# ipastore/glue-factory-colon

Measured on AMD Instinct MI355X. Metric: image-pairs/sec (SuperPoint+LightGlue, 1024 kpts, 640x480), higher is better.
Workload: dtype f32; 1 GPU; SuperPoint-open + LightGlue, 1024 kpts, 640x480 synthetic pairs (BASELINE.json configs[1]); keypoints=1024, parallelism=dp1 (pairs sharded, one final gather), weights=name-seeded seed 0 (no network), pairs_gathered=32, rccl_ranks=1

## Files before the change

### glue-factory-colon_amd/csrc/conv_wino.hip

```cpp
#include "common.h"

#define WT_Y 16
#define WT_X 8
#define WP_R 18
#define WP_C 12
#define WKC 16
#define WPATCH (WP_R * WP_C * WKC)
#define WIM_R 20
#define WIM_C 12
#ifndef WINO_DIAG
#define WINO_DIAG 0
#endif

struct WinoArgs {
  const float* x;
  const float* w;
  const float* bias;
  const float* scale;
  const float* shift;
  float* y;
  int B, H, W, cin, cout, relu;
  int tiles_x, tiles_y;
  const float* w1;
  const float* b1;
  const float* s1;
  const float* t1;
  int xcd_remap;
#if WINO_DIAG & 256
  unsigned long long* diag;
#endif
};
#if WINO_DIAG & 256
static unsigned long long* g_wino_diag = nullptr;
extern "C" void gfc_diag_set_wino_stamps(void* p) { g_wino_diag = (unsigned long long*)p; }
#define WINO_T(v_) const unsigned long long v_ = __builtin_readcyclecounter()
#else
#define WINO_T(v_) do {} while (0)
#endif

__global__ void pack_conv3x3_wino_kernel(const float* __restrict__ w, float* __restrict__ out, int cout, int cin) {
  const int idx = blockIdx.x * blockDim.x + threadIdx.x;
  if (idx >= cout * cin) return;
  const int ci = idx % cin, co = idx / cin;
  double g[3][3];
  for (int r = 0; r < 3; ++r)
    for (int c = 0; c < 3; ++c) g[r][c] = (double)w[((size_t)co * cin + ci) * 9 + r * 3 + c];
  const double G[4][3] = {{1.0, 0.0, 0.0}, {0.5, 0.5, 0.5}, {0.5, -0.5, 0.5}, {0.0, 0.0, 1.0}};
  double t[4][3];
  for (int i = 0; i < 4; ++i)
    for (int c = 0; c < 3; ++c) t[i][c] = G[i][0] * g[0][c] + G[i][1] * g[1][c] + G[i][2] * g[2][c];
  const int nb = co / 64, nt = (co % 64) / 32, l31 = co % 32;
  const int kg = ci / 8, h = (ci % 8) / 4, s = ci % 4;
  const int lane = 32 * h + l31;
  for (int xi = 0; xi < 4; ++xi)
    for (int nu = 0; nu < 4; ++nu) {
      const double u = t[xi][0] * G[nu][0] + t[xi][1] * G[nu][1] + t[xi][2] * G[nu][2];
      const size_t o = ((((((size_t)nb * 4 + xi) * (cin / 8) + kg) * 4 + nu) * 2 + nt) * 64 + lane) * 4 + s;
      out[o] = (float)u;
    }
}

extern "C" int gfc_pack_conv3x3_wino(const float* w_oihw, float* w_packed, int cout, int cin, void* stream) {
  if (!w_oihw || !w_packed || cout <= 0 || cin <= 0 || cout % 64 || cin % WKC) return GFC_ERR_INVALID;
  const int total = cout * cin;
  hipLaunchKernelGGL(pack_conv3x3_wino_kernel, dim3((total + 255) / 256), dim3(256), 0, (hipStream_t)stream, w_oihw,
                     w_packed, cout, cin);
  GFC_LAUNCH_CHECK();
  return GFC_OK;
}

__device__ __forceinline__ float4 f4_axpy(float s, float4 a, float4 b) {
  return make_float4(fmaf(s, a.x, b.x), fmaf(s, a.y, b.y), fmaf(s, a.z, b.z), fmaf(s, a.w, b.w));
}
__device__ __forceinline__ float4 f4_add(float4 a, float4 b) { return make_float4(a.x + b.x, a.y + b.y, a.z + b.z, a.w + b.w); }
__device__ __forceinline__ float4 f4_sub(float4 a, float4 b) { return make_float4(a.x - b.x, a.y - b.y, a.z - b.z, a.w - b.w); }

template <bool POOL, bool STEM>
__global__ __launch_bounds__(256, 2) void conv3x3_wino_kernel(WinoArgs a) {
  extern __shared__ __attribute__((aligned(16))) float smem[];
  float* in_s = smem;
  float* img_s = smem + 16384;
  float* c1_s = img_s + WIM_R * WIM_C;

  const int tid = threadIdx.x, lane = tid & 63;
  const int xi = __builtin_amdgcn_readfirstlane(tid >> 6);
  const int l31 = lane & 31, h = lane >> 5;
  const int cin = a.cin, nchunks = cin / WKC;

  const int ntiles = a.tiles_x * a.tiles_y * a.B;
  const int nitems = ntiles * (a.cout / 64);
  const int nbpair = (a.cout / 64) % 2 == 0 ? 2 : 1;
  int item = blockIdx.x;
  int x0, y0, b, nb;
  const float* xin;
  const float4* wp;
#define WINO_DECODE(w_, x0_, y0_, b_, nb_, xin_, wp_)                                              \
  do {                                                                                             \
    unsigned l_ = a.xcd_remap ? gfc_xcd_chunk((unsigned)(w_), (unsigned)nitems) : (unsigned)(w_);  \
    const int lo_ = (int)(l_ % (unsigned)nbpair);                                                  \
    l_ /= (unsigned)nbpair;                                                                        \
    int t_ = (int)(l_ % (unsigned)ntiles);                                                         \
    nb_ = (int)(l_ / (unsigned)ntiles) * nbpair + lo_;                                             \
    x0_ = (t_ % a.tiles_x) * WT_X;                                                                 \
    t_ /= a.tiles_x;                                                                               \
    y0_ = (t_ % a.tiles_y) * WT_Y;                                                                 \
    b_ = t_ / a.tiles_y;                                                                           \
    xin_ = a.x + (size_t)b_ * a.H * a.W * (STEM ? 1 : cin);                                        \
    wp_ = reinterpret_cast<const float4*>(a.w) + (((size_t)nb_ * 4 + xi) * (cin / 8)) * 512;        \
  } while (0)
  WINO_DECODE(item, x0, y0, b, nb, xin, wp);

  float4 ireg[3];
  int st_off[3];
  int st_gofs[3];
#pragma unroll
  for (int i = 0; i < 3; ++i) {
    const int idx = tid + 256 * i;
    const int pix = idx >> 2, c4 = idx & 3;
    const int py = pix / 10, px = pix - py * 10;
    const int R = (py >> 1) + (py & 1) * 9, C = (px >> 1) + (px & 1) * 5;
    st_off[i] = idx < 720 ? (R * WP_C + C) * WKC + ((c4 ^ (R & 3)) << 2) : -1;
  }
#define WINO_GOFS(y0_, x0_)                                                                        \
  _Pragma("unroll") for (int i_ = 0; i_ < 3; ++i_) {                                               \
    const int py_ = ((tid + 256 * i_) >> 2) / 10, px_ = ((tid + 256 * i_) >> 2) - py_ * 10;        \
    const int gy_ = (y0_) - 1 + py_, gx_ = (x0_) - 1 + px_;                                        \
    const bool in_ = st_off[i_] >= 0 && gy_ >= 0 && gy_ < a.H && gx_ >= 0 && gx_ < a.W;            \
    if constexpr (STEM) st_gofs[i_] = in_ ? (py_ * WIM_C + px_) : -1;  \
    else st_gofs[i_] = in_ ? (int)(((size_t)gy_ * a.W + gx_) * cin + ((tid & 3) << 2)) : -1;       \
  }
#define WINO_LOAD_IN(xin_, chunk_)                                                                \
  _Pragma("unroll") for (int i_ = 0; i_ < 3; ++i_) {                                               \
    float4 v_ = make_float4(0.f, 0.f, 0.f, 0.f);                                                   \
    if (st_gofs[i_] >= 0) v_ = *reinterpret_cast<const float4*>((xin_) + st_gofs[i_] + (chunk_) * WKC); \
    ireg[i_] = v_;                                                                                 \
  }
#define WINO_FILL_IN(chunk_)                                                                      \
  {                                                                                                \
                     \
    const int c0_ = (chunk_) * WKC + ((tid & 3) << 2);                                             \
    float4 wv_[9];                                                                                 \
    _Pragma("unroll") for (int t2_ = 0; t2_ < 9; ++t2_)                                            \
        wv_[t2_] = *reinterpret_cast<const float4*>(c1_s + t2_ * 64 + c0_);                        \
    const float4 b1_ = *reinterpret_cast<const float4*>(c1_s + 576 + c0_);                         \
    const float4 s1_ = *reinterpret_cast<const float4*>(c1_s + 640 + c0_);                         \
    const float4 t1_ = *reinterpret_cast<const float4*>(c1_s + 704 + c0_);                         \
    _Pragma("unroll") for (int i_ = 0; i_ < 3; ++i_) {                                             \
      float4 v_ = make_float4(0.f, 0.f, 0.f, 0.f);   \
      if (st_gofs[i_] >= 0) {                                                                      \
        const float* ip_ = img_s + st_gofs[i_];                                                    \
        _Pragma("unroll") for (int t2_ = 0; t2_ < 9; ++t2_) {                                      \
          const float f_ = ip_[(t2_ / 3) * WIM_C + t2_ % 3];                                       \
          v_.x = fmaf(f_, wv_[t2_].x, v_.x); v_.y = fmaf(f_, wv_[t2_].y, v_.y);                    \
          v_.z = fmaf(f_, wv_[t2_].z, v_.z); v_.w = fmaf(f_, wv_[t2_].w, v_.w);                    \
        }                                                                                          \
        v_.x = fmaxf(v_.x + b1_.x, 0.f) * s1_.x + t1_.x; v_.y = fmaxf(v_.y + b1_.y, 0.f) * s1_.y + t1_.y; \
        v_.z = fmaxf(v_.z + b1_.z, 0.f) * s1_.z + t1_.z; v_.w = fmaxf(v_.w + b1_.w, 0.f) * s1_.w + t1_.w; \
      }                                                                                            \
      ireg[i_] = v_;                                                                               \
    }                                                                                              \
  }
#define WINO_STORE_IN(buf_)                                                                       \
  _Pragma("unroll") for (int i_ = 0; i_ < 3; ++i_)                                                 \
    if (st_off[i_] >= 0) *reinterpret_cast<float4*>(in_s + (buf_) * WPATCH + st_off[i_]) = ireg[i_];
#define WINO_IMG(xin_, y0_, x0_)                                                                   \
  ((tid < WIM_R * WIM_C && (y0_) - 2 + tid / WIM_C >= 0 && (y0_) - 2 + tid / WIM_C < a.H &&        \
    (x0_) - 2 + tid % WIM_C >= 0 && (x0_) - 2 + tid % WIM_C < a.W)                                 \
       ? (xin_)[(size_t)((y0_) - 2 + tid / WIM_C) * a.W + (x0_) - 2 + tid % WIM_C] : 0.f)

  WINO_GOFS(y0, x0);
  if constexpr (STEM) {
    if (tid < WIM_R * WIM_C) img_s[tid] = WINO_IMG(xin, y0, x0);
    for (int i = tid; i < 768; i += 256)
      c1_s[i] = i < 576 ? a.w1[i] : i < 640 ? a.b1[i - 576] : i < 704 ? (a.s1 ? a.s1[i - 640] : 1.f)
                                                                         : (a.t1 ? a.t1[i - 704] : 0.f);
    __syncthreads();
    WINO_FILL_IN(0);
  } else {
    WINO_LOAD_IN(xin, 0);
  }
  float4 bq[4][2];
#pragma unroll
  for (int nu = 0; nu < 4; ++nu)
#pragma unroll
    for (int nt = 0; nt < 2; ++nt) bq[nu][nt] = wp[(nu * 2 + nt) * 64 + lane];

  const int a1 = xi == 0 ? 0 : xi == 2 ? 2 : 1;
  const int a2 = xi == 0 ? 2 : xi == 1 ? 2 : xi == 2 ? 1 : 3;
  const float sg = xi == 1 ? 1.f : -1.f;
  const int ty = l31 >> 2, tx = l31 & 3;
  const int R1 = ty + (a1 >> 1) + (a1 & 1) * 9, R2 = ty + (a2 >> 1) + (a2 & 1) * 9;
  const int o1 = (R1 * WP_C + tx) * WKC + ((h ^ (R1 & 3)) << 2);
  const int o2 = (R2 * WP_C + tx) * WKC + ((h ^ (R2 & 3)) << 2);

#if WINO_DIAG & 256
  unsigned long long d_k = 0, d_x = 0, d_s = 0, d_n = 0, d_epi10 = 0;
  const unsigned long long d_t0 = __builtin_readcyclecounter();
#endif
  while (true) {
  WINO_T(t_a);
  WINO_STORE_IN(0);
  __syncthreads();
  f32x16 acc[4][2];
#pragma unroll
  for (int nu = 0; nu < 4; ++nu)
#pragma unroll
    for (int nt = 0; nt < 2; ++nt)
#pragma unroll
      for (int r = 0; r < 16; ++r) acc[nu][nt][r] = 0.f;
  const int next_item = item + gridDim.x;
  const bool more = !STEM && next_item < nitems;
  int nx0 = 0, ny0 = 0, nbb = 0, nnb = 0;
  const float* nxin = xin;
  const float4* nwp = wp;
  if (more) WINO_DECODE(next_item, nx0, ny0, nbb, nnb, nxin, nwp);

  for (int c = 0; c < nchunks; ++c) {
    const bool has_next = c + 1 < nchunks;
    const float* ps = in_s + (c & 1) * WPATCH;
#pragma unroll
    for (int g = 0; g < 2; ++g) {
      const float* p1 = ps + (g ? (o1 ^ 8) : o1);
      const float* p2 = ps + (g ? (o2 ^ 8) : o2);
      const float4 t0 = f4_axpy(sg, *reinterpret_cast<const float4*>(p2), *reinterpret_cast<const float4*>(p1));
      const float4 t1 = f4_axpy(sg, *reinterpret_cast<const float4*>(p2 + 5 * WKC), *reinterpret_cast<const float4*>(p1 + 5 * WKC));
      const float4 t2 = f4_axpy(sg, *reinterpret_cast<const float4*>(p2 + 1 * WKC), *reinterpret_cast<const float4*>(p1 + 1 * WKC));
      const float4 t3 = f4_axpy(sg, *reinterpret_cast<const float4*>(p2 + 6 * WKC), *reinterpret_cast<const float4*>(p1 + 6 * WKC));
      float4 v[4];
      v[0] = f4_sub(t0, t2);
      v[1] = f4_add(t1, t2);
      v[2] = f4_sub(t2, t1);
      v[3] = f4_sub(t1, t3);
      const int kg_next = 2 * c + g + 1;
      const bool more_b = kg_next < cin / 8 || more;
      const float4* bsrc = kg_next < cin / 8 ? wp + (size_t)kg_next * 512 : nwp;
#pragma unroll
      for (int nu = 0; nu < 4; ++nu) {
        acc[nu][0] = mfma32(v[nu].x, bq[nu][0].x, acc[nu][0]);
        acc[nu][1] = mfma32(v[nu].x, bq[nu][1].x, acc[nu][1]);
        acc[nu][0] = mfma32(v[nu].y, bq[nu][0].y, acc[nu][0]);
        acc[nu][1] = mfma32(v[nu].y, bq[nu][1].y, acc[nu][1]);
        acc[nu][0] = mfma32(v[nu].z, bq[nu][0].z, acc[nu][0]);
        acc[nu][1] = mfma32(v[nu].z, bq[nu][1].z, acc[nu][1]);
        acc[nu][0] = mfma32(v[nu].w, bq[nu][0].w, acc[nu][0]);
        acc[nu][1] = mfma32(v[nu].w, bq[nu][1].w, acc[nu][1]);
        if (more_b) {
          bq[nu][0] = bsrc[(nu * 2 + 0) * 64 + lane];
          bq[nu][1] = bsrc[(nu * 2 + 1) * 64 + lane];
        }
      }
      if (g == 0) {
        if constexpr (STEM) {
          if (has_next) { WINO_FILL_IN(c + 1); }
        } else {
          if (has_next) { WINO_LOAD_IN(xin, c + 1); }
          else if (more) { WINO_GOFS(ny0, nx0); WINO_LOAD_IN(nxin, 0); }
        }
      }
    }
    if (has_next) WINO_STORE_IN((c + 1) & 1);
    __syncthreads();
  }

  WINO_T(t_b);
  float* ex = smem;
#pragma unroll
  for (int nt = 0; nt < 2; ++nt)
#pragma unroll
    for (int r = 0; r < 16; ++r) {
      const float m0 = acc[0][nt][r], m1 = acc[1][nt][r], m2 = acc[2][nt][r], m3 = acc[3][nt][r];
      const int o = acc_row(r, h) * 64 + nt * 32 + l31;
      ex[(xi * 2 + 0) * 2048 + o] = (m0 + m1) + m2;
      ex[(xi * 2 + 1) * 2048 + o] = (m1 - m2) - m3;
    }
  __syncthreads();
  WINO_T(t_c);
  const int q4 = (tid & 15) * 4;
  const int co = nb * 64 + q4;
  const float4 bi = *reinterpret_cast<const float4*>(a.bias + co);
  const float4 sc = a.scale ? *reinterpret_cast<const float4*>(a.scale + co) : make_float4(1.f, 1.f, 1.f, 1.f);
  const float4 sh = a.shift ? *reinterpret_cast<const float4*>(a.shift + co) : make_float4(0.f, 0.f, 0.f, 0.f);
  const bool relu = a.relu != 0;
#pragma unroll
  for (int k = 0; k < 2; ++k) {
    const int tile = (tid >> 4) + 16 * k;
    const float* zp = ex + tile * 64 + q4;
    float4 yv[2][2];
#pragma unroll
    for (int j = 0; j < 2; ++j) {
      const float4 z0 = *reinterpret_cast<const float4*>(zp + (0 * 2 + j) * 2048);
      const float4 z1 = *reinterpret_cast<const float4*>(zp + (1 * 2 + j) * 2048);
      const float4 z2 = *reinterpret_cast<const float4*>(zp + (2 * 2 + j) * 2048);
      const float4 z3 = *reinterpret_cast<const float4*>(zp + (3 * 2 + j) * 2048);
      yv[0][j] = f4_add(f4_add(z0, z1), z2);
      yv[1][j] = f4_sub(f4_sub(z1, z2), z3);
    }
#pragma unroll
    for (int i = 0; i < 2; ++i)
#pragma unroll
      for (int j = 0; j < 2; ++j) {
        float4 t = f4_add(yv[i][j], bi);
        if (relu) t = make_float4(fmaxf(t.x, 0.f), fmaxf(t.y, 0.f), fmaxf(t.z, 0.f), fmaxf(t.w, 0.f));
        yv[i][j] = make_float4(t.x * sc.x + sh.x, t.y * sc.y + sh.y, t.z * sc.z + sh.z, t.w * sc.w + sh.w);
      }
    const int oy = (y0 >> 1) + (tile >> 2), ox = (x0 >> 1) + (tile & 3);
    if constexpr (POOL) {
      const int Ho = a.H >> 1, Wo = a.W >> 1;
      if (oy < Ho && ox < Wo) {
        const float4 u = yv[0][0], v = yv[0][1], w = yv[1][0], z = yv[1][1];
        *reinterpret_cast<float4*>(a.y + (((size_t)b * Ho + oy) * Wo + ox) * a.cout + co) =
            make_float4(fmaxf(fmaxf(u.x, v.x), fmaxf(w.x, z.x)), fmaxf(fmaxf(u.y, v.y), fmaxf(w.y, z.y)),
                        fmaxf(fmaxf(u.z, v.z), fmaxf(w.z, z.z)), fmaxf(fmaxf(u.w, v.w), fmaxf(w.w, z.w)));
      }
    } else {
#pragma unroll
      for (int i = 0; i < 2; ++i)
#pragma unroll
        for (int j = 0; j < 2; ++j) {
          const int gy = 2 * oy + i, gx = 2 * ox + j;
          if (gy < a.H && gx < a.W)
            *reinterpret_cast<float4*>(a.y + (((size_t)b * a.H + gy) * a.W + gx) * a.cout + co) = yv[i][j];
        }
    }
  }
#if WINO_DIAG & 256
  {
    WINO_T(t_d);
    d_k += t_b - t_a; d_x += t_c - t_b; d_s += t_d - t_c; d_n += 1;
    if (d_n == 10) d_epi10 = t_b;
  }
#endif
  if (!more) break;
  item = next_item; x0 = nx0; y0 = ny0; b = nbb; nb = nnb; xin = nxin; wp = nwp;
  __syncthreads();
  }
#if WINO_DIAG & 256
  if (a.diag && lane == 0) {
    unsigned hw, xcc;
    asm volatile("s_getreg_b32 %0, hwreg(HW_REG_HW_ID)" : "=s"(hw));
    asm volatile("s_getreg_b32 %0, hwreg(HW_REG_XCC_ID)" : "=s"(xcc));
    unsigned long long* o = a.diag + ((size_t)blockIdx.x * 4 + xi) * 8;
    o[0] = d_k; o[1] = d_x; o[2] = d_s; o[3] = d_n; o[4] = __builtin_readcyclecounter() - d_t0;
    o[5] = (unsigned long long)hw | ((unsigned long long)(xcc & 0xf) << 32); o[6] = d_t0; o[7] = d_epi10;
  }
#endif
#undef WINO_DECODE
#undef WINO_GOFS
#undef WINO_LOAD_IN
#undef WINO_FILL_IN
#undef WINO_STORE_IN
#undef WINO_IMG
}

template <bool POOL, bool STEM>
static int launch_wino(const WinoArgs& a, hipStream_t st) {
  static_assert(2 * WPATCH <= 16384, "the exchange buffer covers the patch buffers");
  constexpr size_t lds = (size_t)(16384 + (STEM ? WIM_R * WIM_C + 768 : 0)) * sizeof(float);
  static std::atomic<unsigned long long> lds_ok{0};
  if (lds > 64 * 1024) gfc_allow_dynamic_lds((const void*)conv3x3_wino_kernel<POOL, STEM>, lds, lds_ok);
  const long long nitems = (long long)a.tiles_x * a.tiles_y * a.B * (a.cout / 64);
  long long resident = ((long long)gfc_device_cus() * 2) & ~7ll;
  if (resident < 8) resident = 8;
  const long long grid = (STEM || nitems < resident) ? nitems : resident;
  WinoArgs wa = a;
  wa.xcd_remap = nitems >= 16;
#if WINO_DIAG & 256
  wa.diag = g_wino_diag;
#endif
  hipLaunchKernelGGL((conv3x3_wino_kernel<POOL, STEM>), dim3((unsigned)grid), dim3(256), lds, st, wa);
  GFC_LAUNCH_CHECK();
  return GFC_OK;
}

extern "C" int gfc_conv3x3_wino(const float* x, const float* w_wino, const float* bias, const float* scale,
                                const float* shift, float* y, int B, int H, int W, int cin, int cout, int relu, int pool,
                                void* stream) {
  if (!x || !w_wino || !bias || !y || B <= 0 || H <= 0 || W <= 0) return GFC_ERR_INVALID;
  if ((scale == nullptr) != (shift == nullptr)) return GFC_ERR_INVALID;
  if (cin % WKC != 0 || cout % 64 != 0 || cin <= 0 || cout <= 0) return GFC_ERR_UNSUPPORTED;
  if ((long long)H * W * cin >= (1ll << 31)) return GFC_ERR_UNSUPPORTED;
  WinoArgs a = {};
  a.x = x; a.w = w_wino; a.bias = bias; a.scale = scale; a.shift = shift; a.y = y;
  a.B = B; a.H = H; a.W = W; a.cin = cin; a.cout = cout; a.relu = relu;
  a.tiles_x = (W + WT_X - 1) / WT_X;
  a.tiles_y = (H + WT_Y - 1) / WT_Y;
  return pool ? launch_wino<true, false>(a, (hipStream_t)stream) : launch_wino<false, false>(a, (hipStream_t)stream);
}

extern "C" int gfc_sp_stem_wino(const float* image, const float* w1, const float* b1, const float* s1, const float* t1,
                                const float* w2_wino, const float* b2, const float* s2, const float* t2, float* y, int B,
                                int H, int W, void* stream) {
  if (!image || !w1 || !b1 || !w2_wino || !b2 || !y || B <= 0 || H < 2 || W < 2) return GFC_ERR_INVALID;
  if ((s1 == nullptr) != (t1 == nullptr) || (s2 == nullptr) != (t2 == nullptr)) return GFC_ERR_INVALID;
  WinoArgs a = {};
  a.x = image; a.w = w2_wino; a.bias = b2; a.scale = s2; a.shift = t2; a.y = y;
  a.B = B; a.H = H; a.W = W; a.cin = 64; a.cout = 64; a.relu = 1;
  a.w1 = w1; a.b1 = b1; a.s1 = s1; a.t1 = t1;
  a.tiles_x = (W + WT_X - 1) / WT_X;
  a.tiles_y = (H + WT_Y - 1) / WT_Y;
  return launch_wino<true, true>(a, (hipStream_t)stream);
}
```

Baseline: 946.5 image-pairs/sec.

## Flatten batch rows in Winograd conv tiling to avoid partial tiles at image boundaries

Row tiles in the Winograd 3x3 conv are now laid over the concatenated batch×height axis rather than per image, so a 16-row tile can span two images. A zero row is inserted at the seam, the input patch grows to 20 rows, and the A-operand LDS offsets switch per tile depending on the seam position. This is meant to cut wasted work in partially filled tiles when H is not a multiple of 16 (for example 60 or 120 rows at deeper layers). The cost is extra index arithmetic and a larger patch buffer, and the new boundary logic carries correctness risk.

```diff
diff --git a/glue-factory-colon_amd/csrc/conv_wino.hip b/glue-factory-colon_amd/csrc/conv_wino.hip
--- a/glue-factory-colon_amd/csrc/conv_wino.hip
+++ b/glue-factory-colon_amd/csrc/conv_wino.hip
@@ -2,7 +2,10 @@
 
 #define WT_Y 16
 #define WT_X 8
-#define WP_R 18
+#define WP_R 20
+#define WP_ODD 10
+#define WB_MID 256
+#define WZ_NONE 64
 #define WP_C 12
 #define WKC 16
 #define WPATCH (WP_R * WP_C * WKC)
@@ -21,6 +24,9 @@
   float* y;
   int B, H, W, cin, cout, relu;
   int tiles_x, tiles_y;
+  int nrb;
+  int hs;
+  int zb;
   const float* w1;
   const float* b1;
   const float* s1;
@@ -87,14 +93,15 @@
   const int l31 = lane & 31, h = lane >> 5;
   const int cin = a.cin, nchunks = cin / WKC;
 
-  const int ntiles = a.tiles_x * a.tiles_y * a.B;
+  const int ntiles = a.tiles_x * a.nrb;
   const int nitems = ntiles * (a.cout / 64);
   const int nbpair = (a.cout / 64) % 2 == 0 ? 2 : 1;
   int item = blockIdx.x;
   int x0, y0, b, nb;
+  int zr;
   const float* xin;
   const float4* wp;
-#define WINO_DECODE(w_, x0_, y0_, b_, nb_, xin_, wp_)                                              \
+#define WINO_DECODE(w_, x0_, y0_, b_, zr_, nb_, xin_, wp_)                                            \
   do {                                                                                             \
     unsigned l_ = a.xcd_remap ? gfc_xcd_chunk((unsigned)(w_), (unsigned)nitems) : (unsigned)(w_);  \
     const int lo_ = (int)(l_ % (unsigned)nbpair);                                                  \
@@ -103,12 +110,14 @@
     nb_ = (int)(l_ / (unsigned)ntiles) * nbpair + lo_;                                             \
     x0_ = (t_ % a.tiles_x) * WT_X;                                                                 \
     t_ /= a.tiles_x;                                                                               \
-    y0_ = (t_ % a.tiles_y) * WT_Y;                                                                 \
-    b_ = t_ / a.tiles_y;                                                                           \
+     \
+    b_ = (t_ * WT_Y) / a.hs;                                                                       \
+    y0_ = t_ * WT_Y - b_ * a.hs;                                                                   \
+    zr_ = (!STEM && a.H - y0_ < WT_Y && b_ < a.zb) ? a.H - y0_ + 1 : WZ_NONE;                      \
     xin_ = a.x + (size_t)b_ * a.H * a.W * (STEM ? 1 : cin);                                        \
-    wp_ = reinterpret_cast<const float4*>(a.w) + (((size_t)nb_ * 4 + xi) * (cin / 8)) * 512;        \
+    wp_ = reinterpret_cast<const float4*>(a.w) + (((size_t)nb_ * 4 + xi) * (cin / 8)) * 512 + WB_MID; \
   } while (0)
-  WINO_DECODE(item, x0, y0, b, nb, xin, wp);
+  WINO_DECODE(item, x0, y0, b, zr, nb, xin, wp);
 
   float4 ireg[3];
   int st_off[3];
@@ -118,14 +127,18 @@
     const int idx = tid + 256 * i;
     const int pix = idx >> 2, c4 = idx & 3;
     const int py = pix / 10, px = pix - py * 10;
-    const int R = (py >> 1) + (py & 1) * 9, C = (px >> 1) + (px & 1) * 5;
-    st_off[i] = idx < 720 ? (R * WP_C + C) * WKC + ((c4 ^ (R & 3)) << 2) : -1;
-  }
-#define WINO_GOFS(y0_, x0_)                                                                        \
+    const int R = (py >> 1) + (py & 1) * WP_ODD, C = (px >> 1) + (px & 1) * 5;
+    st_off[i] = idx < 760 ? (R * WP_C + C) * WKC + ((c4 ^ (R & 3)) << 2) : -1;
+  }
+#define WINO_GOFS(y0_, x0_, zr_)                                                                      \
   _Pragma("unroll") for (int i_ = 0; i_ < 3; ++i_) {                                               \
     const int py_ = ((tid + 256 * i_) >> 2) / 10, px_ = ((tid + 256 * i_) >> 2) - py_ * 10;        \
-    const int gy_ = (y0_) - 1 + py_, gx_ = (x0_) - 1 + px_;                                        \
-    const bool in_ = st_off[i_] >= 0 && gy_ >= 0 && gy_ < a.H && gx_ >= 0 && gx_ < a.W;            \
+     \
+    const int gy_ = (y0_) - 1 + py_ - (py_ > (zr_) ? 1 : 0), gx_ = (x0_) - 1 + px_;                \
+     \
+    const bool bnd_ = !STEM && (zr_) != WZ_NONE;                                                   \
+    const bool in_ = py_ < (bnd_ ? 19 : 18) && py_ != (zr_) && (unsigned)gy_ < (bnd_ ? 0x7fffffffu : (unsigned)a.H) && \
+                     (unsigned)gx_ < (unsigned)a.W;                                                \
     if constexpr (STEM) st_gofs[i_] = in_ ? (py_ * WIM_C + px_) : -1;  \
     else st_gofs[i_] = in_ ? (int)(((size_t)gy_ * a.W + gx_) * cin + ((tid & 3) << 2)) : -1;       \
   }
@@ -168,7 +181,7 @@
     (x0_) - 2 + tid % WIM_C >= 0 && (x0_) - 2 + tid % WIM_C < a.W)                                 \
        ? (xin_)[(size_t)((y0_) - 2 + tid / WIM_C) * a.W + (x0_) - 2 + tid % WIM_C] : 0.f)
 
-  WINO_GOFS(y0, x0);
+  WINO_GOFS(y0, x0, zr);
   if constexpr (STEM) {
     if (tid < WIM_R * WIM_C) img_s[tid] = WINO_IMG(xin, y0, x0);
     for (int i = tid; i < 768; i += 256)
@@ -183,15 +196,22 @@
 #pragma unroll
   for (int nu = 0; nu < 4; ++nu)
 #pragma unroll
-    for (int nt = 0; nt < 2; ++nt) bq[nu][nt] = wp[(nu * 2 + nt) * 64 + lane];
+    for (int nt = 0; nt < 2; ++nt) bq[nu][nt] = wp[(nu * 2 + nt) * 64 - WB_MID + lane];
 
   const int a1 = xi == 0 ? 0 : xi == 2 ? 2 : 1;
   const int a2 = xi == 0 ? 2 : xi == 1 ? 2 : xi == 2 ? 1 : 3;
   const float sg = xi == 1 ? 1.f : -1.f;
   const int ty = l31 >> 2, tx = l31 & 3;
-  const int R1 = ty + (a1 >> 1) + (a1 & 1) * 9, R2 = ty + (a2 >> 1) + (a2 & 1) * 9;
-  const int o1 = (R1 * WP_C + tx) * WKC + ((h ^ (R1 & 3)) << 2);
-  const int o2 = (R2 * WP_C + tx) * WKC + ((h ^ (R2 & 3)) << 2);
+#define WINO_AOFS(o1_, o2_, zr_)                                                                   \
+  {                                                                                                \
+    const bool s_ = ty >= ((zr_) >> 1);                                                            \
+    const int R1_ = ty + (s_ ? WINO_PROW(a1 + 1) : WINO_PROW(a1));                                 \
+    const int R2_ = ty + (s_ ? WINO_PROW(a2 + 1) : WINO_PROW(a2));                                 \
+    o1_ = R1_ * (WP_C * WKC) + tx * WKC + ((h ^ (R1_ & 3)) << 2);                                  \
+    o2_ = R2_ * (WP_C * WKC) + tx * WKC + ((h ^ (R2_ & 3)) << 2);                                  \
+  }
+#define WINO_PROW(p_) (((p_) >> 1) + ((p_) & 1) * WP_ODD)
+  int o1, o2;
 
 #if WINO_DIAG & 256
   unsigned long long d_k = 0, d_x = 0, d_s = 0, d_n = 0, d_epi10 = 0;
@@ -199,6 +219,7 @@
 #endif
   while (true) {
   WINO_T(t_a);
+  WINO_AOFS(o1, o2, zr);
   WINO_STORE_IN(0);
   __syncthreads();
   f32x16 acc[4][2];
@@ -210,10 +231,10 @@
       for (int r = 0; r < 16; ++r) acc[nu][nt][r] = 0.f;
   const int next_item = item + gridDim.x;
   const bool more = !STEM && next_item < nitems;
-  int nx0 = 0, ny0 = 0, nbb = 0, nnb = 0;
+  int nx0 = 0, ny0 = 0, nbb = 0, nnb = 0, nzr = WZ_NONE;
   const float* nxin = xin;
   const float4* nwp = wp;
-  if (more) WINO_DECODE(next_item, nx0, ny0, nbb, nnb, nxin, nwp);
+  if (more) WINO_DECODE(next_item, nx0, ny0, nbb, nzr, nnb, nxin, nwp);
 
   for (int c = 0; c < nchunks; ++c) {
     const bool has_next = c + 1 < nchunks;
@@ -245,8 +266,8 @@
         acc[nu][0] = mfma32(v[nu].w, bq[nu][0].w, acc[nu][0]);
         acc[nu][1] = mfma32(v[nu].w, bq[nu][1].w, acc[nu][1]);
         if (more_b) {
-          bq[nu][0] = bsrc[(nu * 2 + 0) * 64 + lane];
-          bq[nu][1] = bsrc[(nu * 2 + 1) * 64 + lane];
+          bq[nu][0] = bsrc[(nu * 2 + 0) * 64 - WB_MID + lane];
+          bq[nu][1] = bsrc[(nu * 2 + 1) * 64 - WB_MID + lane];
         }
       }
       if (g == 0) {
@@ -254,7 +275,7 @@
           if (has_next) { WINO_FILL_IN(c + 1); }
         } else {
           if (has_next) { WINO_LOAD_IN(xin, c + 1); }
-          else if (more) { WINO_GOFS(ny0, nx0); WINO_LOAD_IN(nxin, 0); }
+          else if (more) { WINO_GOFS(ny0, nx0, nzr); WINO_LOAD_IN(nxin, 0); }
         }
       }
     }
@@ -281,6 +302,7 @@
   const float4 sc = a.scale ? *reinterpret_cast<const float4*>(a.scale + co) : make_float4(1.f, 1.f, 1.f, 1.f);
   const float4 sh = a.shift ? *reinterpret_cast<const float4*>(a.shift + co) : make_float4(0.f, 0.f, 0.f, 0.f);
   const bool relu = a.relu != 0;
+  const int ylim = (!STEM && zr != WZ_NONE) ? 0x7fffffff : a.H;
 #pragma unroll
   for (int k = 0; k < 2; ++k) {
     const int tile = (tid >> 4) + 16 * k;
@@ -306,7 +328,7 @@
     const int oy = (y0 >> 1) + (tile >> 2), ox = (x0 >> 1) + (tile & 3);
     if constexpr (POOL) {
       const int Ho = a.H >> 1, Wo = a.W >> 1;
-      if (oy < Ho && ox < Wo) {
+      if (oy < (ylim >> 1) && ox < Wo) {
         const float4 u = yv[0][0], v = yv[0][1], w = yv[1][0], z = yv[1][1];
         *reinterpret_cast<float4*>(a.y + (((size_t)b * Ho + oy) * Wo + ox) * a.cout + co) =
             make_float4(fmaxf(fmaxf(u.x, v.x), fmaxf(w.x, z.x)), fmaxf(fmaxf(u.y, v.y), fmaxf(w.y, z.y)),
@@ -318,7 +340,7 @@
 #pragma unroll
         for (int j = 0; j < 2; ++j) {
           const int gy = 2 * oy + i, gx = 2 * ox + j;
-          if (gy < a.H && gx < a.W)
+          if (gy < ylim && gx < a.W)
             *reinterpret_cast<float4*>(a.y + (((size_t)b * a.H + gy) * a.W + gx) * a.cout + co) = yv[i][j];
         }
     }
@@ -331,7 +353,7 @@
   }
 #endif
   if (!more) break;
-  item = next_item; x0 = nx0; y0 = ny0; b = nbb; nb = nnb; xin = nxin; wp = nwp;
+  item = next_item; x0 = nx0; y0 = ny0; b = nbb; zr = nzr; nb = nnb; xin = nxin; wp = nwp;
   __syncthreads();
   }
 #if WINO_DIAG & 256
@@ -346,6 +368,8 @@
 #endif
 #undef WINO_DECODE
 #undef WINO_GOFS
+#undef WINO_AOFS
+#undef WINO_PROW
 #undef WINO_LOAD_IN
 #undef WINO_FILL_IN
 #undef WINO_STORE_IN
@@ -358,7 +382,7 @@
   constexpr size_t lds = (size_t)(16384 + (STEM ? WIM_R * WIM_C + 768 : 0)) * sizeof(float);
   static std::atomic<unsigned long long> lds_ok{0};
   if (lds > 64 * 1024) gfc_allow_dynamic_lds((const void*)conv3x3_wino_kernel<POOL, STEM>, lds, lds_ok);
-  const long long nitems = (long long)a.tiles_x * a.tiles_y * a.B * (a.cout / 64);
+  const long long nitems = (long long)a.tiles_x * a.nrb * (a.cout / 64);
   long long resident = ((long long)gfc_device_cus() * 2) & ~7ll;
   if (resident < 8) resident = 8;
   const long long grid = (STEM || nitems < resident) ? nitems : resident;
@@ -370,6 +394,15 @@
   hipLaunchKernelGGL((conv3x3_wino_kernel<POOL, STEM>), dim3((unsigned)grid), dim3(256), lds, st, wa);
   GFC_LAUNCH_CHECK();
   return GFC_OK;
+}
+
+static bool wino_flat(int B, int H, int W, int cin) {
+  return B > 1 && H >= WT_Y && H % 2 == 0 && H % WT_Y != 0 && (long long)B * H < (1ll << 30) &&
+         ((long long)H + WT_Y + 2) * W * cin < (1ll << 31);
+}
+extern "C" int gfc_conv3x3_wino_row_blocks(int B, int H) {
+  if (B <= 0 || H <= 0) return 0;
+  return wino_flat(B, H, 1, 1) ? (int)(((long long)B * H + WT_Y - 1) / WT_Y) : B * ((H + WT_Y - 1) / WT_Y);
 }
 
 extern "C" int gfc_conv3x3_wino(const float* x, const float* w_wino, const float* bias, const float* scale,
@@ -384,6 +417,10 @@
   a.B = B; a.H = H; a.W = W; a.cin = cin; a.cout = cout; a.relu = relu;
   a.tiles_x = (W + WT_X - 1) / WT_X;
   a.tiles_y = (H + WT_Y - 1) / WT_Y;
+  const bool flat = wino_flat(B, H, W, cin);
+  a.nrb = flat ? (int)(((long long)B * H + WT_Y - 1) / WT_Y) : B * a.tiles_y;
+  a.hs = flat ? H : a.tiles_y * WT_Y;
+  a.zb = flat ? B - 1 : 0;
   return pool ? launch_wino<true, false>(a, (hipStream_t)stream) : launch_wino<false, false>(a, (hipStream_t)stream);
 }
 
@@ -398,5 +435,7 @@
   a.w1 = w1; a.b1 = b1; a.s1 = s1; a.t1 = t1;
   a.tiles_x = (W + WT_X - 1) / WT_X;
   a.tiles_y = (H + WT_Y - 1) / WT_Y;
+  a.nrb = B * a.tiles_y;
+  a.hs = a.tiles_y * WT_Y;
   return launch_wino<true, true>(a, (hipStream_t)stream);
 }
```

New measurement: 948.9 image-pairs/sec, median of 6. Within noise of the previous version (+0.3%).
